# oarodriguez/PhD-QMCLib

Hardware: AMD Instinct MI355X
Metric: walker-steps/sec (higher is better)
Workload: dtype f64

## Files before the change

### phd_qmclib_amd/csrc/qmc_kernels.h

```cpp
#pragma once

#include "qmc_device.h"
#include "qmc_sorted64.h"
#include "qmc_sorted128.h"

#ifndef QMC_SORTED128
#define QMC_SORTED128 1
#endif

static constexpr int BLOCK = 256;

#ifndef QMC_BLOCK64
#define QMC_BLOCK64 64
#endif
template <int G>
struct WalkBlock {
    static constexpr int N = (G == 64) ? QMC_BLOCK64 : BLOCK;
};

#ifndef QMC_XCD_MAP
#define QMC_XCD_MAP 1
#endif
template <int GPB>
__device__ __forceinline__ long long walker_of_block(unsigned b, int grp)
{
    if (QMC_XCD_MAP && GPB == 1)
        return ((long long)(b >> 7) << 7) + ((b & 7u) << 4) + ((b & 127u) >> 3);
    return (long long)b * GPB + grp;
}

template <int G, int P, bool PAD, bool ZC, bool DMC = false>
struct StepLds {
    static constexpr int NROWS =
        DMC ? SortedCot<false, true, false>::ROWS : 5;
    static constexpr int SORTED =
        (QMC_SORTED128 && G == 64 && P == 2 && !ZC)
            ? NROWS * SortedRows<128>::ROW
            : (QMC_SORTED64 && G == 64 && P == 1 && !ZC)
                  ? (NROWS + (QMC_T_LDS ? 1 : 0)) * SortedRows<64>::ROW
                  : 0;
    static constexpr int GENERAL = GroupLds<G, P, ZC>::DOUBLES;
    static constexpr int DOUBLES = SORTED > GENERAL ? SORTED : GENERAL;
};

__device__ __forceinline__ long long qmc_uniform(long long v)
{
    const int lo = __builtin_amdgcn_readfirstlane((int)v);
    const int hi = __builtin_amdgcn_readfirstlane((int)(v >> 32));
    return ((long long)hi << 32) | (unsigned int)lo;
}

#ifndef QMC_LB_P1
#define QMC_LB_P1 7
#endif
#ifndef QMC_LB_DMC_P2
#define QMC_LB_DMC_P2 5
#endif
#define QMC_LB_WAVES , ((G == 64 && P == 1) ? QMC_LB_P1 : 1)
#define QMC_LB_WAVES_DMC , ((G == 64 && P == 1) ? QMC_LB_P1 \
                            : (G == 64 && P == 2 && !ZC) ? QMC_LB_DMC_P2 : 1)
#ifndef QMC_LB_VMC_P2
#define QMC_LB_VMC_P2 4
#endif
#define QMC_LB_WAVES_VMC , ((G == 64 && P == 1) ? QMC_LB_P1 \
                            : (G == 64 && P == 2 && !ZC) ? QMC_LB_VMC_P2 : 1)

#ifndef QMC_VMC_TWO_PASS
#define QMC_VMC_TWO_PASS 1
#endif

#ifndef QMC_DMC_SPARE
#define QMC_DMC_SPARE 1
#endif
template <int P>
struct DmcSpare {
    static constexpr bool ON = QMC_DMC_SPARE && P == 1;
};

#ifndef QMC_RESORT_EVERY
#define QMC_RESORT_EVERY 4
#endif

struct EvalArgs {
    const double *pos;
    double *wf, *energy;
    double *ith, *drift;
    long long nconf;
};

template <int G, int P, bool PAD, bool ZC, typename R = double>
__global__ void __launch_bounds__(WalkBlock<G>::N QMC_LB_WAVES)
evaluate_kernel(const DevModel *__restrict__ mp, EvalArgs a)
{
    const DevModel &m = *mp;
    [[maybe_unused]] constexpr int QMC_SEC_OFF = 0;
    QMC_SECTION("top");
    extern __shared__ double smem[];
    constexpr int GPB = WalkBlock<G>::N / G;
    const int grp = threadIdx.x / G, gl = threadIdx.x % G;
    double *lds = smem + (size_t)grp * GroupLds<G, P, ZC>::DOUBLES;
    const long long w = walker_of_block<GPB>(blockIdx.x, grp);
    const bool active = w < a.nconf;
    if (GPB == 1 && !active) return;
    const long long wr = active ? w : 0;
    const int n = walker_n<G, P, PAD>(m);
    double z[P], z1[P], F[P], ei[P], E, wf;
#pragma unroll
    for (int p = 0; p < P; ++p) {
        int i = lane_particle<G, P, PAD>(m, gl, p);
        z1[p] = (i < n) ? a.pos[wr * n + i] : 0.0;
        z[p] = wrap_box(z1[p], m.L);
    }
    eval_walker<G, P, PAD, true, true, ZC, R>(m, z, z1, gl, lds, F, ei, E, wf);
    if (!active) return;
#pragma unroll
    for (int p = 0; p < P; ++p) {
        int i = lane_particle<G, P, PAD>(m, gl, p);
        if (i < n) {
            if (a.ith) a.ith[w * n + i] = ei[p];
            if (a.drift) a.drift[w * n + i] = F[p];
        }
    }
    if (gl == 0) {
        if (a.wf) a.wf[w] = wf;
        if (a.energy) a.energy[w] = E;
    }
}

struct PrepArgs {
    const double *pos;
    double *drift, *energy;
    long long nconf;
};

template <int G, int P, bool PAD, bool ZC, typename R = double>
__global__ void __launch_bounds__(WalkBlock<G>::N QMC_LB_WAVES)
prepare_kernel(const DevModel *__restrict__ mp, PrepArgs a)
{
    const DevModel &m = *mp;
    [[maybe_unused]] constexpr int QMC_SEC_OFF = 0;
    QMC_SECTION("top");
    extern __shared__ double smem[];
    constexpr int GPB = WalkBlock<G>::N / G;
    const int grp = threadIdx.x / G, gl = threadIdx.x % G;
    double *lds = smem + (size_t)grp * GroupLds<G, P, ZC>::DOUBLES;
    const long long w = walker_of_block<GPB>(blockIdx.x, grp);
    const bool active = w < a.nconf;
    if (GPB == 1 && !active) return;
    const long long wr = active ? w : 0;
    const int n = walker_n<G, P, PAD>(m);
    double z[P], z1[P], F[P], ei[P], E, wf;
#pragma unroll
    for (int p = 0; p < P; ++p) {
        int i = lane_particle<G, P, PAD>(m, gl, p);
        z1[p] = (i < n) ? a.pos[wr * n + i] : 0.0;
        z[p] = wrap_box(z1[p], m.L);
    }
    eval_walker<G, P, PAD, false, false, ZC, R>(m, z, z1, gl, lds, F, ei, E,
                                                wf);
    if (!active) return;
#pragma unroll
    for (int p = 0; p < P; ++p) {
        int i = lane_particle<G, P, PAD>(m, gl, p);
        if (i < n) a.drift[w * n + i] = F[p];
    }
    if (gl == 0) a.energy[w] = E;
}

struct alignas(64) VmcRec {
    double wf;
    double ecarry;
    double sum_e, sum_e2;
    long long n_acc;
    long long spare[3];
};
static_assert(sizeof(VmcRec) == 64, "one record = 8 eight-byte words");
typedef unsigned int VmcRecWords __attribute__((ext_vector_type(16)));
#define QMC_CONST __attribute__((address_space(4)))
__device__ __forceinline__ double vmc_rec_word(const VmcRecWords &r, int k)
{
    return __hiloint2double((int)r[2 * k + 1], (int)r[2 * k]);
}

struct VmcArgs {
    double *pos;
    unsigned short *label;
    VmcRec *rec;
    double *ser_wf, *ser_e;
    unsigned char *ser_stat;
    double *ser_pos;
    const double *tape;
    long long tape_steps;
    long long tape_idx;
    long long W;
    long long y;
    int forced;
    int reset_sums;
    int gaussian;
    unsigned int step;
    unsigned int chain0;
    unsigned long long seed;
    double move_spread;
};

template <int G, int P, bool PAD, bool ZC, bool LEAN, typename R = double,
          bool STEADY = false>
__global__ void __launch_bounds__(WalkBlock<G>::N QMC_LB_WAVES_VMC)
vmc_step_kernel(const DevModel *__restrict__ mp, VmcArgs a)
{
    static_assert(LEAN || !STEADY, "the steady variant is a LEAN kernel");
    const DevModel &m = *mp;
    [[maybe_unused]] constexpr int QMC_SEC_OFF = 0;
    QMC_SECTION("top");
    extern __shared__ double smem[];
    constexpr int GPB = WalkBlock<G>::N / G;
    const int grp = threadIdx.x / G, gl = threadIdx.x % G;
    static_assert(StepLds<G, P, PAD, ZC>::DOUBLES >= GroupLds<G, P, ZC>::DOUBLES,
                  "eval_walker is the fallback on the same LDS region");
    double *lds = smem + (size_t)grp * StepLds<G, P, PAD, ZC>::DOUBLES;
    const long long w = walker_of_block<GPB>(blockIdx.x, grp);
    const bool active = w < a.W;
    if (GPB == 1 && !active) return;
    const long long wr = active ? w : 0;
    const int n = walker_n<G, P, PAD>(m);
    const unsigned int slot = a.chain0 + (unsigned int)wr;
    const bool forced = !STEADY && a.forced != 0;
    const bool reset_sums = !STEADY && a.reset_sums != 0;

    const long long wl = (G == 64) ? qmc_uniform(wr) : wr;
    double wf_cur, e_cur, se = 0.0, se2 = 0.0;
    long long na = 0;
    if constexpr (G == 64) {
        const VmcRecWords r = *(const QMC_CONST VmcRecWords *)(a.rec + wl);
        wf_cur = vmc_rec_word(r, 0);
        e_cur = vmc_rec_word(r, 1);
        se = vmc_rec_word(r, 2);
        se2 = vmc_rec_word(r, 3);
        na = __double_as_longlong(vmc_rec_word(r, 4));
        if (reset_sums) { se = 0.0; se2 = 0.0; na = 0; }
    } else {
        wf_cur = a.rec[wl].wf;
        e_cur = a.rec[wl].ecarry;
    }

    QMC_SECTION("load+philox+wrap");
    double zn[P];
    int labn[P];
    double ua = 1.0;
    unsigned int aw0 = 0u, aw1 = 0u;
    bool has0 = false, has1 = false;
    bool outside = false;
#pragma unroll
    for (int p = 0; p < P; ++p) {
        int i = lane_particle<G, P, PAD>(m, gl, p);
        const double zp = (i < n) ? a.pos[wr * n + i] : 0.0;
        labn[p] = (i < n) ? (int)a.label[wr * n + i] : i;
        const unsigned li = (unsigned)labn[p];
        double d = 0.0;
        if (!forced && i < n) {
            if (!LEAN && a.tape) {
                double tv = a.tape[(wr * a.tape_steps + a.tape_idx) * (n + 1) + li];
                d = a.gaussian ? a.move_spread * tv
                               : (tv - 0.5) * a.move_spread;
            } else if (!LEAN && a.gaussian) {
                double g0, g1;
                philox_normal2(a.seed, slot, a.step, li, STREAM_VMC_MOVE, g0,
                               g1);
                d = a.move_spread * g0;
            } else {
                uint32_t w0, w1;
                vmc_move_block(a.seed, slot, a.step, li, w0, w1);
                d = vmc_move_unit(w0) * a.move_spread;
                if (li == 0u) { aw0 = w1; has0 = true; }
                if (li == 1u || n == 1) { aw1 = w1; has1 = true; }
            }
        }
        zn[p] = wrap_box(zp + d, m.L);
        if (forced) outside = outside || zn[p] != zp;
    }
    QMC_SECTION("resort");
    constexpr bool S64 = QMC_SORTED64 && G == 64 && P == 1 && !ZC;
    constexpr bool S128 = QMC_SORTED128 && G == 64 && P == 2 && !ZC;
    bool fast = false;
    if (forced)
        outside = __builtin_amdgcn_ballot_w64(outside) != 0ull;
    if constexpr (S64) {
        fast = !m.is_ideal && !outside &&
               sort_lanes64(zn[0], labn[0], gl, PAD ? n : 64) &&
               (PAD ? far_partner_ok_ring(m, zn[0], gl, n)
                    : far_partner_ok64(m, zn[0], gl));
    } else if constexpr (S128) {
        fast = !m.is_ideal && !outside && (!PAD || (n & 1) == 0) &&
               sort_rows128(zn, labn, gl, PAD ? n / 2 : 64) &&
               (PAD ? far_partner_ok_ring128(m, zn, gl, n / 2)
                    : far_partner_ok128(m, zn, gl));
    }
    if constexpr (S64 || S128) {
        if (!fast && !m.is_ideal && gl == 0 && active)
            atomicAdd(m.diag, 1ull);
    } else if constexpr (G == 64 && P == 1 && QMC_LINEAR_ORDER) {
        if (!forced) {
            anchor_seam(zn[0], labn[0], n);
            if ((a.step % QMC_RESORT_EVERY) == 0)
                resort_linear<G>(zn[0], labn[0], gl,
                                 a.step / QMC_RESORT_EVERY, n);
        }
    } else if constexpr (SlotMap<G, P>::CONSECUTIVE && QMC_LINEAR_ORDER) {
        if (!forced) {
            anchor_seam_rows<P>(zn, labn, n);
            if ((a.step % QMC_RESORT_EVERY) == 0)
                resort_linear_rows<P>(zn, labn, gl, a.step / QMC_RESORT_EVERY, n);
        }
    } else if (!forced && (a.step % QMC_RESORT_EVERY) == 0)
        resort_step<G, P>(zn, labn, gl, a.step / QMC_RESORT_EVERY, n, m.L,
                          m.half_L, lanes_in_use<G, PAD>(m));
    constexpr bool TWO_PASS = QMC_VMC_TWO_PASS && (G == 64);
    double F[P], ei[P], e_new = 0.0, wf_new;
    if (S64 && fast) {
        if constexpr (S64)
            eval_sorted64<R, true, !TWO_PASS, false, PAD>(
                m, zn[0], gl, lds, F[0], e_new, wf_new);
    } else if (S128 && fast) {
        if constexpr (S128)
            eval_sorted128<R, true, !TWO_PASS, false, PAD>(m, zn, gl, lds, F,
                                                           e_new, wf_new);
    } else {
        double z1[P];
#pragma unroll
        for (int p = 0; p < P; ++p) {
            int i = lane_particle<G, P, PAD>(m, gl, p);
            z1[p] = (outside && i < n) ? a.pos[wr * n + i] : zn[p];
        }
        if constexpr (TWO_PASS)
            eval_walker<G, P, PAD, true, false, ZC, R, false, false>(
                m, zn, z1, gl, lds, F, ei, e_new, wf_new);
        else
            eval_walker<G, P, PAD, true, false, ZC, R>(m, zn, z1, gl, lds, F,
                                                       ei, e_new, wf_new);
    }
    QMC_SECTION("metropolis+store");
    if (!forced) {
        if (!LEAN && a.tape) {
            ua = a.tape[(wr * a.tape_steps + a.tape_idx) * (n + 1) + n];
        } else if (!LEAN && a.gaussian) {
            double u1;
            philox_uniform2(a.seed, slot, a.step, 0u, STREAM_VMC_ACCEPT, ua,
                            u1);
        } else {
            const unsigned long long bal0 = __ballot(has0);
            const unsigned long long bal1 = __ballot(has1);
            unsigned int hi, lo;
            if (G == 64) {
                const int src0 = __builtin_amdgcn_readfirstlane(
                    (int)__ffsll((long long)bal0) - 1) & 63;
                const int src1 = __builtin_amdgcn_readfirstlane(
                    (int)__ffsll((long long)bal1) - 1) & 63;
                hi = (unsigned)__builtin_amdgcn_readlane((int)aw0, src0);
                lo = (unsigned)__builtin_amdgcn_readlane((int)aw1, src1);
            } else {
                const int base = (threadIdx.x & 63) - gl;
                const unsigned long long gmask = (1ull << (G & 63)) - 1ull;
                const int src0 = base + ((__ffsll((long long)((bal0 >> base) &
                                                              gmask)) - 1) & (G - 1));
                const int src1 = base + ((__ffsll((long long)((bal1 >> base) &
                                                              gmask)) - 1) & (G - 1));
                hi = (unsigned)__shfl((int)aw0, src0, 64);
                lo = (unsigned)__shfl((int)aw1, src1, 64);
            }
            ua = u53(hi, lo);
        }
    }
    if (!active) return;
    bool acc = forced || ua <= 0.0 || wf_new > wf_cur;
    if (!acc) acc = wf_new > 0.5 * log_pos(ua) + wf_cur;
    if (G == 64) acc = __builtin_amdgcn_readfirstlane((int)acc) != 0;
    if (acc) {
        if constexpr (TWO_PASS) {
            QMC_SECTION("energy_pass");
            QMC_SECTION_PHASE(QMC_NSEC / 2);
            double wf_unused;
            if (S64 && fast) {
                if constexpr (S64)
                    eval_sorted64<R, false, true, true, PAD>(
                        m, zn[0], gl, lds, F[0], e_new, wf_unused);
            } else if (S128 && fast) {
                if constexpr (S128)
                    eval_sorted128<R, false, true, true, PAD>(
                        m, zn, gl, lds, F, e_new, wf_unused);
            } else {
                double z1[P];
#pragma unroll
                for (int p = 0; p < P; ++p) {
                    int i = lane_particle<G, P, PAD>(m, gl, p);
                    z1[p] = (outside && i < n) ? a.pos[wr * n + i] : zn[p];
                }
                eval_walker<G, P, PAD, false, false, ZC, R, true, true>(
                    m, zn, z1, gl, lds, F, ei, e_new, wf_unused);
            }
            QMC_SECTION_PHASE(0);
            QMC_SECTION("store");
        }
#pragma unroll
        for (int p = 0; p < P; ++p) {
            int i = lane_particle<G, P, PAD>(m, gl, p);
            if (i < n && !forced) {
                a.pos[w * n + i] = zn[p];
                a.label[w * n + i] = (unsigned short)labn[p];
            }
        }
        wf_cur = wf_new;
        e_cur = e_new;
    }
    if (!LEAN && a.ser_pos) {
#pragma unroll
        for (int p = 0; p < P; ++p) {
            int i = lane_particle<G, P, PAD>(m, gl, p);
            if (i < n) {
                const bool moved = acc && !forced;
                const int lb = moved ? labn[p] : (int)a.label[w * n + i];
                a.ser_pos[(a.y * a.W + w) * n + lb] =
                    moved ? zn[p] : a.pos[w * n + i];
            }
        }
    }
    if (G == 64) {
        const double sum1 = se + e_cur;
        const double sum2 = fma(e_cur, e_cur, se2);
        const long long na1 = qmc_uniform(na + (acc ? 1 : 0));
        double v = __longlong_as_double((gl == 4) ? na1 : 0ll);
        v = (gl == 0) ? wf_cur : v;
        v = (gl == 1) ? e_cur : v;
        v = (gl == 2) ? sum1 : v;
        v = (gl == 3) ? sum2 : v;
        if (gl < 8) reinterpret_cast<double *>(a.rec + wl)[gl] = v;
    }
    if (gl == 0) {
        if (G != 64) {
            VmcRec *r = a.rec + w;
            if (!reset_sums) { se = r->sum_e; se2 = r->sum_e2; na = r->n_acc; }
            r->wf = wf_cur;
            r->ecarry = e_cur;
            r->sum_e = se + e_cur;
            r->sum_e2 = fma(e_cur, e_cur, se2);
            r->n_acc = na + (acc ? 1 : 0);
        }
        if (!LEAN) {
            if (a.ser_wf) a.ser_wf[a.y * a.W + w] = wf_cur;
            if (a.ser_e) a.ser_e[a.y * a.W + w] = e_cur;
            if (a.ser_stat) a.ser_stat[a.y * a.W + w] = acc ? 1 : 0;
        }
    }
    QMC_SECTION("end");
}

struct DmcCtl {
    long long prev_nw;
    long long nw;
    double ref_energy;
    double total_energy, total_weight;
    double e_t, w_t;
    long long spare_nw;
    unsigned int step;
    unsigned int pad;
};

struct EvolveArgs {
    const double *ppos, *pdrift, *penergy;
    double *cpos, *cdrift, *cenergy, *cweight;
    const unsigned short *plabel;
    unsigned short *clabel;
    double *eslot;
    const long long *ref;
    const DmcCtl *ctl;
    const double *g_tape;
    double *spare;
    long long maxw;
    double dt, sigma;
    unsigned long long seed;
    unsigned int slot0;
    int fix_stale;
};

template <int G, int P, bool PAD, bool ZC, typename R = double>
__global__ void __launch_bounds__(WalkBlock<G>::N QMC_LB_WAVES_DMC)
dmc_evolve_kernel(const DevModel *__restrict__ mp, EvolveArgs a)
{
    const DevModel &m = *mp;
    [[maybe_unused]] constexpr int QMC_SEC_OFF = 0;
    extern __shared__ double smem[];
    constexpr int GPB = WalkBlock<G>::N / G;
    const int grp = threadIdx.x / G, gl = threadIdx.x % G;
    static_assert(StepLds<G, P, PAD, ZC, true>::DOUBLES >=
                      GroupLds<G, P, ZC>::DOUBLES,
                  "eval_walker is the fallback on the same LDS region");
    double *lds = smem + (size_t)grp * StepLds<G, P, PAD, ZC, true>::DOUBLES;
    const long long s = walker_of_block<GPB>(blockIdx.x, grp);
    const long long nw = a.ctl->nw;
    if ((GPB == 1 ? s : (long long)blockIdx.x * GPB) >= nw) return;
    QMC_SECTION("top");
    const bool active = s < nw;
    const long long sr = active ? s : 0;
    const int n = walker_n<G, P, PAD>(m);
    const unsigned int step = a.ctl->step;
    const double ref_energy = a.ctl->ref_energy;
    const long long spare_nw = a.ctl->spare_nw;
    const long long su = (G == 64) ? qmc_uniform(sr) : sr;
    const long long par = a.ref[su];
    double e_par = 0.0, e_slot = 0.0;
    if (G == 64) {
        e_par = a.penergy[par];
        e_slot = a.eslot[su];
    }

    QMC_SECTION("load+philox+wrap");
    double z[P];
    int lab[P];
#pragma unroll
    for (int p = 0; p < P; ++p) {
        int i = lane_particle<G, P, PAD>(m, gl, p);
        double zz = 0.0;
        lab[p] = i;
        if (i < n) {
            double z0 = a.ppos[par * n + i];
            double f0 = a.pdrift[par * n + i];
            const int li = (int)a.plabel[par * n + i];
            lab[p] = li;
            double g;
            if (a.g_tape) {
                g = a.g_tape[sr * n + li];
            } else if (DmcSpare<P>::ON && (step & 1u) && sr < spare_nw) {
                g = a.spare[sr * n + li];
            } else {
                double g0, g1;
                dmc_normal2(a.seed, a.slot0 + (unsigned)sr, step >> 1,
                            (unsigned)li, g0, g1);
                g = (step & 1u) ? g1 : g0;
                if (DmcSpare<P>::ON && !(step & 1u) && active)
                    a.spare[sr * n + li] = g1;
            }
            double zn = z0 + 2 * f0 * a.dt + a.sigma * g;
            zz = wrap_box(zn, m.L);
        }
        z[p] = zz;
    }
    QMC_SECTION("resort");
    constexpr bool S64 = QMC_SORTED64 && G == 64 && P == 1 && !ZC;
    constexpr bool S128 = QMC_SORTED128 && G == 64 && P == 2 && !ZC;
    bool fast = false;
    if constexpr (S64) {
        fast = !m.is_ideal && sort_lanes64(z[0], lab[0], gl, PAD ? n : 64) &&
               (PAD ? far_partner_ok_ring(m, z[0], gl, n)
                    : far_partner_ok64(m, z[0], gl));
    } else if constexpr (S128) {
        fast = !m.is_ideal && (!PAD || (n & 1) == 0) &&
               sort_rows128(z, lab, gl, PAD ? n / 2 : 64) &&
               (PAD ? far_partner_ok_ring128(m, z, gl, n / 2)
                    : far_partner_ok128(m, z, gl));
    }
    if constexpr (S64 || S128) {
        if (!fast && !m.is_ideal && gl == 0 && active)
            atomicAdd(m.diag, 1ull);
    } else if constexpr (G == 64 && P == 1 && QMC_LINEAR_ORDER) {
        anchor_seam(z[0], lab[0], n);
        if ((step % QMC_RESORT_EVERY) == 0)
            resort_linear<G>(z[0], lab[0], gl, step / QMC_RESORT_EVERY, n);
    } else if constexpr (SlotMap<G, P>::CONSECUTIVE && QMC_LINEAR_ORDER) {
        anchor_seam_rows<P>(z, lab, n);
        if ((step % QMC_RESORT_EVERY) == 0)
            resort_linear_rows<P>(z, lab, gl, step / QMC_RESORT_EVERY, n);
    } else if ((step % QMC_RESORT_EVERY) == 0)
        resort_step<G, P>(z, lab, gl, step / QMC_RESORT_EVERY, n, m.L,
                          m.half_L, lanes_in_use<G, PAD>(m));
#pragma unroll
    for (int p = 0; p < P; ++p) {
        int i = lane_particle<G, P, PAD>(m, gl, p);
        if (active && i < n) {
            a.cpos[s * n + i] = z[p];
            a.clabel[s * n + i] = (unsigned short)lab[p];
        }
    }
    double F[P], ei[P], e_next, wf;
    if (S64 && fast) {
        if constexpr (S64)
            eval_sorted64<R, false, true, false, PAD>(m, z[0], gl, lds, F[0],
                                                      e_next, wf);
    } else if (S128 && fast) {
        if constexpr (S128)
            eval_sorted128<R, false, true, false, PAD>(m, z, gl, lds, F,
                                                       e_next, wf);
    } else
        eval_walker<G, P, PAD, false, false, ZC, R>(m, z, z, gl, lds, F, ei,
                                                    e_next, wf);
    QMC_SECTION("weight+store");
    if (!active) return;
#pragma unroll
    for (int p = 0; p < P; ++p) {
        int i = lane_particle<G, P, PAD>(m, gl, p);
        if (i < n) a.cdrift[s * n + i] = F[p];
    }
    if (gl == 0) {
        if (G != 64) { e_par = a.penergy[par]; e_slot = a.eslot[s]; }
        double e_old = a.fix_stale ? e_par : e_slot;
        double mean_energy = (e_next + e_old) / 2;
// ... 7 lines not shown
```

### phd_qmclib_amd/csrc/qmcwalk.hip

```cpp
#include "qmc_inst.h"
#include "qmc_kernels_misc.h"
#include "../../include/qmcwalk.h"

#include <cmath>
#include <cstdio>
#include <cstdlib>
#include <cstring>
#include <algorithm>
#include <string>
#include <vector>

static thread_local std::string g_err;

static int fail(const std::string &msg)
{
    g_err = msg;
    return 1;
}

#define HIP_TRY(expr)                                                        \
    do {                                                                     \
        hipError_t _e = (expr);                                              \
        if (_e != hipSuccess)                                                \
            return fail(std::string(#expr) + ": " + hipGetErrorString(_e));  \
// ... 50 lines not shown


static int pick_shape(int n, int &G, int &P, bool &pad)
{
    if (n < 1) return 1;
    if (const char *env = getenv("QMCWALK_SHAPE")) {
        int g = 0, p = 0;
        if (sscanf(env, "%d,%d", &g, &p) == 2 && n <= g * p) {
            static const int ok[][2] = { {16, 1}, {16, 2}, {32, 2}, {64, 1},
                                         {64, 2}, {64, 4}, {64, 8} };
            for (auto &s : ok)
                if (s[0] == g && s[1] == p) {
                    G = g; P = p; pad = (n != G * P);
                    return 0;
                }
        }
    }
    if (n <= 16) { G = 16; P = 1; }
    else if (n <= 32) { G = 16; P = 2; }
    else if (n <= 64) { G = 64; P = 1; }
    else if (n <= 128) { G = 64; P = 2; }
    else if (n <= 256) { G = 64; P = 4; }
    else if (n <= 512) { G = 64; P = 8; }
    else return 1;
    pad = (n != G * P);
    return 0;
}

#define QMC_EXTERN_TU(name) QMC_TU_##name(extern)
QMC_FOR_ALL_TUS(QMC_EXTERN_TU)
#undef QMC_EXTERN_TU

template <template <int, int, bool, bool> class L, typename... A>
static int dispatch_shape(const qmc_engine *e, A &&...args)
{
    const bool zc = e->dm.zclass != 0;
#define QMC_CASE(g, p)                                                        \
    if (e->G == g && e->P == p) {                                             \
        constexpr bool always = L<g, p, true, false>::want_mask(p);           \
        if (always || e->pad) {                                               \
            if (zc) return L<g, p, true, true>::run(e, args...);              \
            return L<g, p, true, false>::run(e, args...);                     \
        }                                                                     \
        if constexpr (!always) {                                              \
            if (zc) return L<g, p, false, true>::run(e, args...);             \
            return L<g, p, false, false>::run(e, args...);                    \
        }                                                                     \
    }
    QMC_FOR_ALL_SHAPES(QMC_CASE)
#undef QMC_CASE
    return fail("unsupported boson_number");
}

template <int G, int P, bool ZC>
static size_t lds_bytes()
{
    return (size_t)(WalkBlock<G>::N / G) * GroupLds<G, P, ZC>::DOUBLES *
           sizeof(double);
}

template <int G, int P, bool PAD, bool ZC, bool DMC = false>
static size_t step_lds_bytes()
{
    return (size_t)(WalkBlock<G>::N / G) *
           StepLds<G, P, PAD, ZC, DMC>::DOUBLES * sizeof(double);
}

template <typename K>
static void allow_lds(K kernel, size_t bytes)
{
    if (bytes > 48 * 1024)
        (void)hipFuncSetAttribute((const void *)kernel,
                                  hipFuncAttributeMaxDynamicSharedMemorySize,
                                  (int)bytes);
}

template <int G>
static unsigned grid_for(long long nwalkers)
{
    const long long gpb = WalkBlock<G>::N / G;
    long long blocks = (nwalkers + gpb - 1) / gpb;
    if (QMC_XCD_MAP && gpb == 1) blocks = (blocks + 127) / 128 * 128;
    return (unsigned)blocks;
}

template <int G, bool ZC>
static constexpr bool has_fast() { return G == 64 && !ZC; }

template <int G, int P, bool PAD, bool ZC>
struct LaunchEval {
    static constexpr bool want_mask(int np) { return np >= 4; }
    static int run(const qmc_engine *e, const EvalArgs &a)
    {
        if (a.nconf <= 0) return 0;
        const size_t lds = lds_bytes<G, P, ZC>();
        if constexpr (has_fast<G, ZC>()) {
            if (e->fast) {
                allow_lds(evaluate_kernel<G, P, PAD, ZC, float>, lds);
                hipLaunchKernelGGL((evaluate_kernel<G, P, PAD, ZC, float>),
                                   dim3(grid_for<G>(a.nconf)), dim3(WalkBlock<G>::N),
                                   lds, e->stream, e->dm_dev, a);
                HIP_TRY(hipGetLastError());
                return 0;
            }
        }
        allow_lds(evaluate_kernel<G, P, PAD, ZC>, lds);
        hipLaunchKernelGGL((evaluate_kernel<G, P, PAD, ZC>),
                           dim3(grid_for<G>(a.nconf)), dim3(WalkBlock<G>::N),
                           lds, e->stream, e->dm_dev, a);
        HIP_TRY(hipGetLastError());
        return 0;
    }
};

template <int G, int P, bool PAD, bool ZC>
struct LaunchPrep {
    static constexpr bool want_mask(int np) { return np >= 4; }
    static int run(const qmc_engine *e, const PrepArgs &a)
    {
        if (a.nconf <= 0) return 0;
        const size_t lds = lds_bytes<G, P, ZC>();
        if constexpr (has_fast<G, ZC>()) {
            if (e->fast) {
                allow_lds(prepare_kernel<G, P, PAD, ZC, float>, lds);
                hipLaunchKernelGGL((prepare_kernel<G, P, PAD, ZC, float>),
                                   dim3(grid_for<G>(a.nconf)), dim3(WalkBlock<G>::N),
                                   lds, e->stream, e->dm_dev, a);
                HIP_TRY(hipGetLastError());
                return 0;
            }
        }
        allow_lds(prepare_kernel<G, P, PAD, ZC>, lds);
        hipLaunchKernelGGL((prepare_kernel<G, P, PAD, ZC>),
                           dim3(grid_for<G>(a.nconf)), dim3(WalkBlock<G>::N),
                           lds, e->stream, e->dm_dev, a);
        HIP_TRY(hipGetLastError());
        return 0;
    }
};

template <int G, int P, bool PAD, bool ZC>
struct LaunchVmc {
    static constexpr bool want_mask(int np) { return np >= 4; }
    template <typename R, bool LEAN, bool STEADY>
    static void launch(const qmc_engine *e, const VmcArgs &a, size_t lds)
    {
        allow_lds(vmc_step_kernel<G, P, PAD, ZC, LEAN, R, STEADY>, lds);
        hipLaunchKernelGGL((vmc_step_kernel<G, P, PAD, ZC, LEAN, R, STEADY>),
                           dim3(grid_for<G>(a.W)), dim3(WalkBlock<G>::N), lds,
                           e->stream, e->dm_dev, a);
    }
    template <typename R>
    static void launch(const qmc_engine *e, const VmcArgs &a, size_t lds,
                       bool lean)
    {
        if (lean && !a.forced && !a.reset_sums)
            launch<R, true, true>(e, a, lds);
        else if (lean)
            launch<R, true, false>(e, a, lds);
        else
            launch<R, false, false>(e, a, lds);
    }
    static int run(const qmc_engine *e, const VmcArgs &a)
    {
        const size_t lds = step_lds_bytes<G, P, PAD, ZC>();
        const bool lean = !a.tape && !a.gaussian && !a.ser_wf && !a.ser_e &&
                          !a.ser_stat && !a.ser_pos;
        ProfScope prof(e);
        if constexpr (has_fast<G, ZC>()) {
            if (e->fast) {
                launch<float>(e, a, lds, lean);
                HIP_TRY(hipGetLastError());
                return 0;
            }
        }
        launch<double>(e, a, lds, lean);
        HIP_TRY(hipGetLastError());
        return 0;
    }
};

template <int G, int P, bool PAD, bool ZC>
struct LaunchEvolve {
    static constexpr bool want_mask(int np) { return np >= 4; }
    static int run(const qmc_engine *e, const EvolveArgs &a)
    {
        const size_t lds = step_lds_bytes<G, P, PAD, ZC, true>();
        ProfScope prof(e);
        if constexpr (has_fast<G, ZC>()) {
            if (e->fast) {
                allow_lds(dmc_evolve_kernel<G, P, PAD, ZC, float>, lds);
                hipLaunchKernelGGL((dmc_evolve_kernel<G, P, PAD, ZC, float>),
                                   dim3(grid_for<G>(a.maxw)), dim3(WalkBlock<G>::N),
                                   lds, e->stream, e->dm_dev, a);
                HIP_TRY(hipGetLastError());
                return 0;
            }
        }
        allow_lds(dmc_evolve_kernel<G, P, PAD, ZC>, lds);
        hipLaunchKernelGGL((dmc_evolve_kernel<G, P, PAD, ZC>),
                           dim3(grid_for<G>(a.maxw)), dim3(WalkBlock<G>::N),
                           lds, e->stream, e->dm_dev, a);
        HIP_TRY(hipGetLastError());
        return 0;
    }
};

static void build_dev_model(const qmc_model_params &p, DevModel &d)
{
    memset(&d, 0, sizeof(d));
    d.n = (int)p.boson_number;
    d.is_free = p.is_free != 0;
    d.is_ideal = p.is_ideal != 0;
    d.defects_sep = (int)(p.defects_sep > 0 ? p.defects_sep : 1);
    d.L = p.supercell_size;
    d.half_L = 0.5 * d.L;
    d.rm = fabs(p.tbf_contact_cutoff);
    d.L_minus_rm = d.L - d.rm;
    d.two_over_L = 2.0 / d.L;
    d.k2_2pi = p.param_k2 * (2.0 / QMC_PI);
    d.k2 = p.param_k2;
    d.k2sq = d.k2 * d.k2;
    double phi = p.param_k2 * p.param_r_off;
    d.cphi = cos(phi);
    d.sphi = sin(phi);
    d.sec_cut = -1;
    d.am_cphi = fabs(p.param_am) * d.cphi;
    d.am_sphi = fabs(p.param_am) * d.sphi;
    d.m_k2cphi = -d.k2 * d.cphi;
    d.k2sphi = d.k2 * d.sphi;
    double th = p.param_k2 * d.L;
    d.cth = cos(th);
    d.sth = fabs(sin(th));
    d.sth_sign = sin(th) < 0.0 ? (int)0x80000000u : 0;
    d.sth_signed = sin(th);
    d.sp_ok = (!d.is_ideal && th > 0.0 && th < QMC_PI - 1e-9 &&
               d.rm < d.half_L) ? 1 : 0;
    d.sp_xlo = -d.k2 * sin(d.k2 * d.rm - phi);
    d.sp_xhi = d.k2 * sin(phi);
    d.sp_cos = cos(d.k2 * d.rm);
    {
        const double ang[4] = { -phi, phi, phi - th, th - phi };
        for (int v = 0; v < 4; ++v) {
            d.var_cos[v] = cos(ang[v]);
            d.var_sin[v] = sin(ang[v]);
        }
        d.m_k2 = -d.k2;
    }
    d.sin_rm = (d.rm >= d.half_L) ? 1.0 : sin(QMC_PI * d.rm / d.L);
#ifdef QMC_ABLATION
    if (const char *env = getenv("QMCWALK_ABL_SINRM")) d.sin_rm = atof(env);
#endif
    d.zclass = d.rm > 0.45 * d.L;
    double pi_L = QMC_PI / d.L;
    d.a_long = pi_L * p.param_beta;
    d.b_long = pi_L * pi_L * p.param_beta;
    d.a_long_sq = d.a_long * d.a_long;
    d.m_k2_over_a = d.a_long != 0.0 ? -d.k2 / d.a_long : 0.0;
    d.m_a_over_k2 = d.k2 != 0.0 ? -d.a_long / d.k2 : 0.0;
    d.beta = p.param_beta;
    d.inv_beta = p.param_beta != 0.0 ? 1.0 / p.param_beta : 0.0;
    d.one_minus_beta = 1.0 - p.param_beta;
    d.log_am = log(fabs(p.param_am));
    d.z_a = 1.0 / (1.0 + p.lattice_ratio);
    d.z_b = p.lattice_ratio / (1.0 + p.lattice_ratio);
    d.k1 = p.param_k1;
    d.k1_2pi = p.param_k1 * (2.0 / QMC_PI);
    d.kp1 = p.param_kp1;
    d.e0 = p.param_e0;
    d.v0 = p.lattice_depth;
    d.v0d = p.defect_magnitude;
    d.uniform_barrier = (d.defects_sep == 1 || d.v0d == d.v0) ? 1 : 0;
    d.v_barrier = (d.defects_sep == 1) ? d.v0d : d.v0;
    d.k1_half = 0.5 * p.param_k1;
    d.v0_minus_e0 = p.lattice_depth - p.param_e0;
    if (!d.is_free) {
        double sh = sinh(0.5 * sqrt(d.v0 - d.e0) * d.z_b);
        d.cf = sqrt(1 + d.v0 / d.e0 * sh * sh);
    } else {
        d.cf = 1.0;
    }
}

static void ob_exact(const DevModel &d, long double zc, bool barrier,
                     long double &ldz, long double &logf)
{
    if (barrier) {
        const long double x = (long double)d.kp1 *
                              (zc - 1.0L + 0.5L * (long double)d.z_b);
        ldz = (long double)d.kp1 * tanhl(x);
        logf = logl(coshl(x));
    } else {
        const long double x = (long double)d.k1 *
                              (zc - 0.5L * (long double)d.z_a);
        ldz = -(long double)d.k1 * tanl(x);
        logf = logl((long double)d.cf * cosl(x));
    }
}

template <int DEG, typename F>
static void ob_fit(F f, long double a, long double h, double *coef)
{
    constexpr int K = DEG + 1;
    long double A[K][K + 1];
    for (int j = 0; j < K; ++j) {
        const long double t = 0.5L * (1.0L + cosl(3.14159265358979323846264338L *
                                                  (2 * j + 1) / (2.0L * K)));
        long double pw = 1.0L;
        for (int k = 0; k < K; ++k) { A[j][k] = pw; pw *= t; }
        A[j][K] = f(a + h * t);
    }
    for (int c = 0; c < K; ++c) {
        int piv = c;
        for (int r = c + 1; r < K; ++r)
            if (fabsl(A[r][c]) > fabsl(A[piv][c])) piv = r;
        for (int k = 0; k <= K; ++k) std::swap(A[c][k], A[piv][k]);
        for (int r = c + 1; r < K; ++r) {
            const long double g = A[r][c] / A[c][c];
            for (int k = c; k <= K; ++k) A[r][k] -= g * A[c][k];
        }
    }
    for (int r = K - 1; r >= 0; --r) {
        long double v = A[r][K];
        for (int k = r + 1; k < K; ++k) v -= A[r][k] * (long double)coef[k];
        coef[r] = (double)(v / A[r][r]);
    }
}

static double ob_horner(const double *c, int deg, double t)
// ... 680 lines not shown
                       v->ecarry);
    HIP_TRY(hipGetLastError());
    HIP_TRY(hipStreamSynchronize(e->stream));
    v->step = 0;
    v->yield_initial = 1;
    v->tape_used = 0;
    return 0;
}

extern "C" int qmc_vmc_get_state(qmc_vmc *v, double *pos, double *wf,
                                 double *ecarry)
{
    if (!v) return fail("qmc_vmc_get_state: null argument");
    qmc_engine *e = v->eng;
    HIP_TRY(hipSetDevice(e->device));
    const size_t W = (size_t)v->W, n = (size_t)e->dm.n;
    std::vector<double> lane_pos;
    std::vector<unsigned short> label;
    if (pos) {
        lane_pos.resize(W * n);
        label.resize(W * n);
        HIP_TRY(hipMemcpyAsync(lane_pos.data(), v->pos, W * n * sizeof(double),
                               hipMemcpyDeviceToHost, e->stream));
        HIP_TRY(hipMemcpyAsync(label.data(), v->label,
                               W * n * sizeof(unsigned short),
                               hipMemcpyDeviceToHost, e->stream));
    }
    if (wf) HIP_TRY(hipMemcpyAsync(wf, v->wf, W * sizeof(double),
                                   hipMemcpyDeviceToHost, e->stream));
    if (ecarry) HIP_TRY(hipMemcpyAsync(ecarry, v->ecarry, W * sizeof(double),
                                       hipMemcpyDeviceToHost, e->stream));
    HIP_TRY(hipStreamSynchronize(e->stream));
    if (pos)
        for (size_t w = 0; w < W; ++w)
            for (size_t i = 0; i < n; ++i)
                pos[w * n + label[w * n + i]] = lane_pos[w * n + i];
    return 0;
}

extern "C" int qmc_vmc_set_tape(qmc_vmc *v, const double *tape, int64_t steps)
{
    if (!v) return fail("qmc_vmc_set_tape: null argument");
    qmc_engine *e = v->eng;
    HIP_TRY(hipSetDevice(e->device));
    if (v->tape) { hipFree(v->tape); v->tape = nullptr; }
    v->tape_steps = 0;
    v->tape_used = 0;
    if (!tape || steps <= 0) return 0;
    size_t cnt = (size_t)v->W * (size_t)steps * (size_t)(e->dm.n + 1);
    if (dev_alloc(&v->tape, cnt)) return 1;
    HIP_TRY(hipMemcpy(v->tape, tape, cnt * sizeof(double),
                      hipMemcpyHostToDevice));
    v->tape_steps = steps;
    return 0;
}

extern "C" int qmc_vmc_state_dev(qmc_vmc *v, double **pos, double **wf)
{
    if (!v) return fail("null argument");
    if (pos) *pos = v->pos;
    if (wf) *wf = v->wf;
    return 0;
}

extern "C" int qmc_vmc_ssf(qmc_vmc *v, int32_t num_modes, double *out)
{
    if (!v || !out) return fail("qmc_vmc_ssf: null argument");
    if (num_modes <= 0 || num_modes > EST_MAXK)
        return fail("qmc_vmc_ssf: num_modes must be in [1, 256]");
    qmc_engine *e = v->eng;
    HIP_TRY(hipSetDevice(e->device));
    const int M = num_modes;
    if (M > v->ssf_cap) {
        if (v->ssf_partial) { hipFree(v->ssf_partial); hipFree(v->ssf_out); }
        v->ssf_partial = v->ssf_out = nullptr;
        if (dev_alloc(&v->ssf_partial, (size_t)EST_BLOCKS * M * 3) ||
            dev_alloc(&v->ssf_out, (size_t)M * 3))
            return 1;
        v->ssf_cap = M;
    }
    EstArgs a;
    a.ppos = v->pos; a.ref = nullptr; a.ctl = nullptr;
    a.aux_prev = nullptr; a.aux_act = nullptr; a.partial = v->ssf_partial;
    a.maxw = v->W; a.step_idx = 0; a.pfw = 0; a.n = e->dm.n; a.K = M;
    a.pure = 0; a.scale = 4.0 / e->dm.L;
    if (M <= 64) {
        const size_t lds = (size_t)(BLOCK / 64) * SsfShape<8>::WAVE_DOUBLES *
                           sizeof(double);
        allow_lds(dmc_ssf_mfma_kernel<8>, lds);
        hipLaunchKernelGGL(dmc_ssf_mfma_kernel<8>, dim3(EST_BLOCKS),
                           dim3(BLOCK), lds, e->stream, a);
    } else {
        const size_t lds = (size_t)(BLOCK / 64) * SsfShape<16>::WAVE_DOUBLES *
                           sizeof(double);
        allow_lds(dmc_ssf_mfma_kernel<16>, lds);
        hipLaunchKernelGGL(dmc_ssf_mfma_kernel<16>, dim3(EST_BLOCKS),
                           dim3(BLOCK), lds, e->stream, a);
    }
    hipLaunchKernelGGL(est_reduce_kernel, dim3((M * 3 + 31) / 32), dim3(256), 0,
                       e->stream, v->ssf_partial, EST_BLOCKS, M * 3, 1.0,
                       v->ssf_out);
    HIP_TRY(hipGetLastError());
    HIP_TRY(hipMemcpyAsync(out, v->ssf_out, (size_t)M * 3 * sizeof(double),
                           hipMemcpyDeviceToHost, e->stream));
    HIP_TRY(hipStreamSynchronize(e->stream));
    return 0;
}

extern "C" int qmc_vmc_block_sums_dev(qmc_vmc *v, double **se, double **se2,
                                      int64_t **na)
{
    if (!v) return fail("null argument");
    if (se) *se = v->sum_e;
    if (se2) *se2 = v->sum_e2;
    if (na) *na = (int64_t *)v->n_acc;
    return 0;
}

extern "C" int qmc_vmc_run_block(qmc_vmc *v, int64_t nyield, double *sum_e,
                                 double *sum_e2, int64_t *n_acc,
                                 double *ser_wf, double *ser_e,
                                 uint8_t *ser_stat, double *ser_pos)
{
    if (!v) return fail("qmc_vmc_run_block: null argument");
    if (nyield <= 0) return fail("qmc_vmc_run_block: nyield must be >= 1");
    qmc_engine *e = v->eng;
    HIP_TRY(hipSetDevice(e->device));
    const size_t W = (size_t)v->W, ny = (size_t)nyield;
    const long long real = nyield - (v->yield_initial ? 1 : 0);
    if (v->tape && v->tape_used + real > v->tape_steps)
        return fail("qmc_vmc_run_block: tape exhausted");
    double *dwf = nullptr, *de = nullptr;
    unsigned char *dst = nullptr;
    double *dpos = nullptr;
    if ((ser_pos && dev_alloc(&dpos, ny * W * (size_t)e->dm.n)) ||
        (ser_wf && dev_alloc(&dwf, ny * W)) ||
        (ser_e && dev_alloc(&de, ny * W)) ||
        (ser_stat && dev_alloc(&dst, ny * W))) {
        if (dpos) hipFree(dpos);
        if (dwf) hipFree(dwf);
        if (de) hipFree(de);
        if (dst) hipFree(dst);
        return 1;
    }
    VmcArgs a;
    a.pos = v->pos; a.label = v->label; a.rec = v->rec;
    a.ser_wf = dwf; a.ser_e = de; a.ser_stat = dst; a.ser_pos = dpos;
    a.tape = v->tape;
    a.tape_steps = v->tape_steps;
    a.W = v->W;
    a.gaussian = v->p.gaussian;
    a.chain0 = v->p.chain0;
    a.seed = v->p.rng_seed; a.move_spread = v->p.move_spread;
    for (long long y = 0; y < nyield; ++y) {
        a.y = y;
        a.forced = (y == 0 && v->yield_initial) ? 1 : 0;
        a.reset_sums = (y == 0) ? 1 : 0;
        a.step = v->step;
        a.tape_idx = v->tape_used;
        int rc = dispatch_shape<LaunchVmc>(e, a);
        if (rc) return rc;
        if (!a.forced) { v->step += 1; v->tape_used += 1; }
    }
    v->yield_initial = 0;
    hipLaunchKernelGGL(vmc_unpack_kernel, dim3((unsigned)((W + BLOCK - 1) / BLOCK)),
                       dim3(BLOCK), 0, e->stream, v->rec, v->W, v->wf, v->ecarry,
                       v->sum_e, v->sum_e2, v->n_acc);
    HIP_TRY(hipGetLastError());
    bool need_sync = false;
    if (sum_e) { HIP_TRY(hipMemcpyAsync(sum_e, v->sum_e, W * sizeof(double),
                 hipMemcpyDeviceToHost, e->stream)); need_sync = true; }
    if (sum_e2) { HIP_TRY(hipMemcpyAsync(sum_e2, v->sum_e2, W * sizeof(double),
                  hipMemcpyDeviceToHost, e->stream)); need_sync = true; }
    if (n_acc) { HIP_TRY(hipMemcpyAsync(n_acc, v->n_acc, W * sizeof(int64_t),
                 hipMemcpyDeviceToHost, e->stream)); need_sync = true; }
    if (ser_wf) { HIP_TRY(hipMemcpyAsync(ser_wf, dwf, ny * W * sizeof(double),
                  hipMemcpyDeviceToHost, e->stream)); need_sync = true; }
    if (ser_e) { HIP_TRY(hipMemcpyAsync(ser_e, de, ny * W * sizeof(double),
                 hipMemcpyDeviceToHost, e->stream)); need_sync = true; }
    if (ser_stat) { HIP_TRY(hipMemcpyAsync(ser_stat, dst, ny * W,
                    hipMemcpyDeviceToHost, e->stream)); need_sync = true; }
    if (ser_pos) { HIP_TRY(hipMemcpyAsync(ser_pos, dpos,
                   ny * W * (size_t)e->dm.n * sizeof(double),
                   hipMemcpyDeviceToHost, e->stream)); need_sync = true; }
    if (need_sync) HIP_TRY(hipStreamSynchronize(e->stream));
    if (dpos) hipFree(dpos);
    if (dwf) hipFree(dwf);
    if (de) hipFree(de);
    if (dst) hipFree(dst);
    return 0;
}

struct qmc_dmc {
    qmc_engine *eng = nullptr;
    qmc_dmc_params p;
    long long maxw = 0;
    int nblocks = 0;
    double *pos[2] = { nullptr, nullptr }, *drift[2] = { nullptr, nullptr };
    unsigned short *label[2] = { nullptr, nullptr };
    double *energy[2] = { nullptr, nullptr }, *weight[2] = { nullptr, nullptr };
    int cur = 0;
    double *eslot = nullptr;
    double *spare = nullptr;
    long long *ref = nullptr;
    int *count = nullptr;
    long long *block_tot = nullptr, *block_off = nullptr;
    double *block_esum = nullptr;
    DmcCtl *ctl = nullptr;
    double *ser_e = nullptr, *ser_w = nullptr, *ser_ref = nullptr,
           *ser_acc = nullptr;
    unsigned long long *ser_nw = nullptr;
    long long ser_cap = 0, ser_len = 0;
    double *u_tape = nullptr, *g_tape = nullptr;
    std::vector<long long> u_off, g_off;
    long long tape_step = 0;
    bool stepped = false;
    std::vector<double> init_weight;
    bool sums_pending = false;
    double global_target = 0.0;
    qmc_dmc_est_params est;
    bool have_est = false;
    double *ssf_aux[2] = { nullptr, nullptr };
    double *dens_aux[2] = { nullptr, nullptr };
    double *est_partial = nullptr;
    double *iter_ssf = nullptr, *iter_dens = nullptr;
    size_t iter_ssf_cap = 0, iter_dens_cap = 0;
    long long est_block_steps = 0;
    int est_last_act = 1;
};

static int dmc_reserve_series(qmc_dmc *d, long long nsteps)
{
    if (nsteps <= d->ser_cap) return 0;
    if (d->ser_e) hipFree(d->ser_e);
    if (d->ser_w) hipFree(d->ser_w);
    if (d->ser_ref) hipFree(d->ser_ref);
    if (d->ser_acc) hipFree(d->ser_acc);
    if (d->ser_nw) hipFree(d->ser_nw);
    d->ser_e = d->ser_w = d->ser_ref = d->ser_acc = nullptr;
    d->ser_nw = nullptr;
    d->ser_cap = 0;
    if (dev_alloc(&d->ser_e, nsteps) || dev_alloc(&d->ser_w, nsteps) ||
        dev_alloc(&d->ser_ref, nsteps) || dev_alloc(&d->ser_acc, nsteps) ||
        dev_alloc(&d->ser_nw, nsteps)) {
        if (d->ser_e) hipFree(d->ser_e);
        if (d->ser_w) hipFree(d->ser_w);
        if (d->ser_ref) hipFree(d->ser_ref);
        if (d->ser_acc) hipFree(d->ser_acc);
        if (d->ser_nw) hipFree(d->ser_nw);
        d->ser_e = d->ser_w = d->ser_ref = d->ser_acc = nullptr;
        d->ser_nw = nullptr;
        return 1;
    }
    d->ser_cap = nsteps;
    return 0;
}

extern "C" void qmc_dmc_destroy(qmc_dmc *d);

extern "C" int qmc_dmc_create(qmc_engine *e, const qmc_dmc_params *p,
                              qmc_dmc **out)
{
    if (!e || !p || !out) return fail("qmc_dmc_create: null argument");
    if (p->max_num_walkers <= 0 || p->target_num_walkers <= 0)
        return fail("qmc_dmc_create: walker counts must be positive");
    if (!(p->time_step > 0)) return fail("qmc_dmc_create: time_step <= 0");
    HIP_TRY(hipSetDevice(e->device));
    qmc_dmc *d = new qmc_dmc();
    d->eng = e;
    d->p = *p;
    d->maxw = p->max_num_walkers;
    d->nblocks = (int)((d->maxw + BR_TILE - 1) / BR_TILE);
    d->global_target = (double)p->target_num_walkers;
    const size_t W = (size_t)d->maxw, n = (size_t)e->dm.n;
    int rc = 0;
    for (int b = 0; b < 2 && !rc; ++b) {
        rc |= dev_alloc(&d->pos[b], W * n) || dev_alloc(&d->drift[b], W * n) ||
              dev_alloc(&d->label[b], W * n) ||
              dev_alloc(&d->energy[b], W) || dev_alloc(&d->weight[b], W);
    }
    const bool need_spare = QMC_DMC_SPARE && e->P == 1;
    rc = rc || dev_alloc(&d->eslot, W) ||
         (need_spare && dev_alloc(&d->spare, W * n)) ||
         dev_alloc(&d->ref, W) ||
         dev_alloc(&d->count, W) || dev_alloc(&d->block_tot, d->nblocks) ||
         dev_alloc(&d->block_off, d->nblocks) ||
         dev_alloc(&d->block_esum, d->nblocks) || dev_alloc(&d->ctl, 1);
    if (rc) { qmc_dmc_destroy(d); return 1; }
    HIP_TRY(hipMemset(d->ctl, 0, sizeof(DmcCtl)));
    HIP_TRY(hipMemset(d->ref, 0, W * sizeof(long long)));
    HIP_TRY(hipMemset(d->eslot, 0, W * sizeof(double)));
    *out = d;
    return 0;
}

extern "C" void qmc_dmc_destroy(qmc_dmc *d)
{
    if (!d) return;
    hipSetDevice(d->eng->device);
    for (int b = 0; b < 2; ++b) {
        hipFree(d->pos[b]); hipFree(d->drift[b]); hipFree(d->label[b]);
        hipFree(d->energy[b]); hipFree(d->weight[b]);
    }
    hipFree(d->eslot); hipFree(d->spare); hipFree(d->ref); hipFree(d->count);
    hipFree(d->block_tot); hipFree(d->block_off); hipFree(d->block_esum);
    hipFree(d->ctl);
    if (d->ser_e) { hipFree(d->ser_e); hipFree(d->ser_w); hipFree(d->ser_ref);
                    hipFree(d->ser_acc); hipFree(d->ser_nw); }
    if (d->u_tape) hipFree(d->u_tape);
    if (d->g_tape) hipFree(d->g_tape);
    for (int k = 0; k < 2; ++k) {
        if (d->ssf_aux[k]) hipFree(d->ssf_aux[k]);
        if (d->dens_aux[k]) hipFree(d->dens_aux[k]);
    }
    if (d->est_partial) hipFree(d->est_partial);
// ... 798 lines not shown
```

Before: 711.0 million.

## Fuse steady-state VMC steps into one kernel launch with register-resident walker state

In the steady lean VMC path, one kernel launch now runs all remaining steps for a walker in a loop. Positions, labels, energy and accumulator sums stay in registers across steps and are written back to global memory only once at the end. The acceptance random words are taken from the lanes holding labels 0 and 1 using precomputed source lanes and readlane, instead of a ballot on every step. This removes the per-step launch overhead and the per-step global load/store of walker state, at the cost of longer-running kernels, more register pressure, and an opaque-asm trick to keep the compiler from hoisting work out of the loop.

Measured after the change: 762.7 million, median of 6. 1.07x the previous value.

```diff
diff --git a/phd_qmclib_amd/csrc/qmc_kernels.h b/phd_qmclib_amd/csrc/qmc_kernels.h
--- a/phd_qmclib_amd/csrc/qmc_kernels.h
+++ b/phd_qmclib_amd/csrc/qmc_kernels.h
@@ -48,6 +48,49 @@
     const int lo = __builtin_amdgcn_readfirstlane((int)v);
     const int hi = __builtin_amdgcn_readfirstlane((int)(v >> 32));
     return ((long long)hi << 32) | (unsigned int)lo;
+}
+__device__ __forceinline__ int qmc_opaque(int v)
+{
+    asm volatile("" : "+v"(v));
+    return v;
+}
+__device__ __forceinline__ double qmc_uniform_f64(double v)
+{
+    return __longlong_as_double(qmc_uniform(__double_as_longlong(v)));
+}
+__device__ __forceinline__ double qmc_lane_f64(double v, int k)
+{
+    const long long b = __double_as_longlong(v);
+    const int lo = __builtin_amdgcn_readlane((int)b, k);
+    const int hi = __builtin_amdgcn_readlane((int)(b >> 32), k);
+    return __longlong_as_double(((long long)hi << 32) | (unsigned int)lo);
+}
+
+template <int P>
+__device__ __forceinline__ void vmc_accept_lanes(const int (&lab)[P], int n,
+                                                 int &src0, int &src1)
+{
+    src0 = 0;
+    src1 = 0;
+#pragma unroll
+    for (int p = 0; p < P; ++p) {
+        const unsigned long long b0 = __ballot(lab[p] == 0);
+        const unsigned long long b1 = __ballot(lab[p] == 1);
+        if (b0) src0 = ((int)__ffsll((long long)b0) - 1) | (p << 6);
+        if (b1) src1 = ((int)__ffsll((long long)b1) - 1) | (p << 6);
+    }
+    if (n == 1) src1 = src0;
+}
+template <int P>
+__device__ __forceinline__ unsigned int vmc_read_slot(const uint32_t (&wd)[P],
+                                                      int src)
+{
+    unsigned int r = 0u;
+#pragma unroll
+    for (int p = 0; p < P; ++p)
+        if ((src >> 6) == p)
+            r = (unsigned)__builtin_amdgcn_readlane((int)wd[p], src & 63);
+    return r;
 }
 
 #ifndef QMC_LB_P1
@@ -194,6 +237,7 @@
     long long tape_idx;
     long long W;
     long long y;
+    unsigned int nsteps;
     int forced;
     int reset_sums;
     int gaussian;
@@ -201,6 +245,16 @@
     unsigned int chain0;
     unsigned long long seed;
     double move_spread;
+};
+
+#ifndef QMC_VMC_FUSED
+#define QMC_VMC_FUSED 1
+#endif
+template <int G, int P, bool ZC>
+struct VmcFused {
+    static constexpr bool ON =
+        QMC_VMC_FUSED && G == 64 && !ZC &&
+        ((P == 1 && QMC_SORTED64) || (P == 2 && QMC_SORTED128));
 };
 
 template <int G, int P, bool PAD, bool ZC, bool LEAN, typename R = double,
@@ -243,6 +297,26 @@
         e_cur = a.rec[wl].ecarry;
     }
 
+    constexpr bool FUSED = STEADY && VmcFused<G, P, ZC>::ON;
+    double zc[P];
+    int labc[P];
+    int src0 = 0, src1 = 0;
+    if constexpr (FUSED) {
+#pragma unroll
+        for (int p = 0; p < P; ++p) {
+            int i = lane_particle<G, P, PAD>(m, gl, p);
+            zc[p] = (i < n) ? a.pos[wr * n + i] : 0.0;
+            labc[p] = (i < n) ? (int)a.label[wr * n + i] : i;
+        }
+        vmc_accept_lanes<P>(labc, n, src0, src1);
+    }
+    bool any_acc = false;
+    const unsigned int nst = FUSED ? a.nsteps : 1u;
+    bool acc = false;
+    [[maybe_unused]] const int gl_top = gl;
+    for (unsigned int s = 0; s < nst; ++s) {
+    const unsigned int step = a.step + s;
+    const int gl = FUSED ? qmc_opaque(gl_top) : gl_top;
     QMC_SECTION("load+philox+wrap");
     double zn[P];
     int labn[P];
@@ -250,11 +324,19 @@
     unsigned int aw0 = 0u, aw1 = 0u;
     bool has0 = false, has1 = false;
     bool outside = false;
-#pragma unroll
-    for (int p = 0; p < P; ++p) {
+    [[maybe_unused]] uint32_t wacc[P];
+#pragma unroll
+    for (int p = 0; p < P; ++p) {
+        wacc[p] = 0u;
         int i = lane_particle<G, P, PAD>(m, gl, p);
-        const double zp = (i < n) ? a.pos[wr * n + i] : 0.0;
-        labn[p] = (i < n) ? (int)a.label[wr * n + i] : i;
+        double zp;
+        if constexpr (FUSED) {
+            zp = zc[p];
+            labn[p] = labc[p];
+        } else {
+            zp = (i < n) ? a.pos[wr * n + i] : 0.0;
+            labn[p] = (i < n) ? (int)a.label[wr * n + i] : i;
+        }
         const unsigned li = (unsigned)labn[p];
         double d = 0.0;
         if (!forced && i < n) {
@@ -264,19 +346,27 @@
                                : (tv - 0.5) * a.move_spread;
             } else if (!LEAN && a.gaussian) {
                 double g0, g1;
-                philox_normal2(a.seed, slot, a.step, li, STREAM_VMC_MOVE, g0,
+                philox_normal2(a.seed, slot, step, li, STREAM_VMC_MOVE, g0,
                                g1);
                 d = a.move_spread * g0;
             } else {
                 uint32_t w0, w1;
-                vmc_move_block(a.seed, slot, a.step, li, w0, w1);
+                vmc_move_block(a.seed, slot, step, li, w0, w1);
                 d = vmc_move_unit(w0) * a.move_spread;
-                if (li == 0u) { aw0 = w1; has0 = true; }
-                if (li == 1u || n == 1) { aw1 = w1; has1 = true; }
+                if constexpr (FUSED) {
+                    wacc[p] = w1;
+                } else {
+                    if (li == 0u) { aw0 = w1; has0 = true; }
+                    if (li == 1u || n == 1) { aw1 = w1; has1 = true; }
+                }
             }
         }
         zn[p] = wrap_box(zp + d, m.L);
         if (forced) outside = outside || zn[p] != zp;
+    }
+    if constexpr (FUSED) {
+        aw0 = vmc_read_slot<P>(wacc, src0);
+        aw1 = vmc_read_slot<P>(wacc, src1);
     }
     QMC_SECTION("resort");
     constexpr bool S64 = QMC_SORTED64 && G == 64 && P == 1 && !ZC;
@@ -339,12 +429,14 @@
                                                        ei, e_new, wf_new);
     }
     QMC_SECTION("metropolis+store");
-    if (!forced) {
+    if (FUSED) {
+        ua = u53(aw0, aw1);
+    } else if (!forced) {
         if (!LEAN && a.tape) {
             ua = a.tape[(wr * a.tape_steps + a.tape_idx) * (n + 1) + n];
         } else if (!LEAN && a.gaussian) {
             double u1;
-            philox_uniform2(a.seed, slot, a.step, 0u, STREAM_VMC_ACCEPT, ua,
+            philox_uniform2(a.seed, slot, step, 0u, STREAM_VMC_ACCEPT, ua,
                             u1);
         } else {
             const unsigned long long bal0 = __ballot(has0);
@@ -371,9 +463,16 @@
         }
     }
     if (!active) return;
-    bool acc = forced || ua <= 0.0 || wf_new > wf_cur;
-    if (!acc) acc = wf_new > 0.5 * log_pos(ua) + wf_cur;
-    if (G == 64) acc = __builtin_amdgcn_readfirstlane((int)acc) != 0;
+    if constexpr (FUSED) {
+        const double w0 = qmc_uniform_f64(wf_new);
+        acc = ua <= 0.0 || w0 > wf_cur;
+        if (!acc) acc = w0 > 0.5 * log_pos(ua) + wf_cur;
+        acc = __builtin_amdgcn_readfirstlane((int)acc) != 0;
+    } else {
+        acc = forced || ua <= 0.0 || wf_new > wf_cur;
+        if (!acc) acc = wf_new > 0.5 * log_pos(ua) + wf_cur;
+        if (G == 64) acc = __builtin_amdgcn_readfirstlane((int)acc) != 0;
+    }
     if (acc) {
         if constexpr (TWO_PASS) {
             QMC_SECTION("energy_pass");
@@ -400,16 +499,45 @@
             QMC_SECTION_PHASE(0);
             QMC_SECTION("store");
         }
-#pragma unroll
-        for (int p = 0; p < P; ++p) {
-            int i = lane_particle<G, P, PAD>(m, gl, p);
-            if (i < n && !forced) {
-                a.pos[w * n + i] = zn[p];
-                a.label[w * n + i] = (unsigned short)labn[p];
+        if constexpr (FUSED) {
+#pragma unroll
+            for (int p = 0; p < P; ++p) {
+                zc[p] = zn[p];
+                labc[p] = labn[p];
             }
-        }
-        wf_cur = wf_new;
-        e_cur = e_new;
+            vmc_accept_lanes<P>(labc, n, src0, src1);
+            any_acc = true;
+        } else {
+#pragma unroll
+            for (int p = 0; p < P; ++p) {
+                int i = lane_particle<G, P, PAD>(m, gl, p);
+                if (i < n && !forced) {
+                    a.pos[w * n + i] = zn[p];
+                    a.label[w * n + i] = (unsigned short)labn[p];
+                }
+            }
+        }
+        if (!FUSED) {
+            wf_cur = wf_new;
+            e_cur = e_new;
+        }
+    }
+    if constexpr (FUSED) {
+        if (acc) {
+            wf_cur = qmc_uniform_f64(wf_new);
+            const double e2 = qmc_lane_f64(e_new, 2);
+            const double e3 = qmc_lane_f64(e_new, 3);
+            e_cur = qmc_lane_f64(e_new, 1);
+            se = se + e2;
+            se2 = fma(e3, e3, se2);
+            na = na + 1;
+        } else {
+            se = se + e_cur;
+            se2 = fma(e_cur, e_cur, se2);
+        }
+        se = qmc_uniform_f64(se);
+        se2 = qmc_uniform_f64(se2);
+        continue;
     }
     if (!LEAN && a.ser_pos) {
 #pragma unroll
@@ -449,6 +577,26 @@
             if (a.ser_e) a.ser_e[a.y * a.W + w] = e_cur;
             if (a.ser_stat) a.ser_stat[a.y * a.W + w] = acc ? 1 : 0;
         }
+    }
+    }
+    if constexpr (FUSED) {
+        QMC_SECTION("fused_store");
+        if (any_acc) {
+#pragma unroll
+            for (int p = 0; p < P; ++p) {
+                int i = lane_particle<G, P, PAD>(m, gl, p);
+                if (i < n) {
+                    a.pos[w * n + i] = zc[p];
+                    a.label[w * n + i] = (unsigned short)labc[p];
+                }
+            }
+        }
+        double v = __longlong_as_double((gl == 4) ? qmc_uniform(na) : 0ll);
+        v = (gl == 0) ? wf_cur : v;
+        v = (gl == 1) ? e_cur : v;
+        v = (gl == 2) ? se : v;
+        v = (gl == 3) ? se2 : v;
+        if (gl < 8) reinterpret_cast<double *>(a.rec + wl)[gl] = v;
     }
     QMC_SECTION("end");
 }
diff --git a/phd_qmclib_amd/csrc/qmcwalk.hip b/phd_qmclib_amd/csrc/qmcwalk.hip
--- a/phd_qmclib_amd/csrc/qmcwalk.hip
+++ b/phd_qmclib_amd/csrc/qmcwalk.hip
@@ -226,29 +226,31 @@
     }
     template <typename R>
     static void launch(const qmc_engine *e, const VmcArgs &a, size_t lds,
-                       bool lean)
+                       bool lean, bool steady)
     {
-        if (lean && !a.forced && !a.reset_sums)
+        if (steady)
             launch<R, true, true>(e, a, lds);
         else if (lean)
             launch<R, true, false>(e, a, lds);
         else
             launch<R, false, false>(e, a, lds);
     }
-    static int run(const qmc_engine *e, const VmcArgs &a)
+    static int run(const qmc_engine *e, const VmcArgs &a, long long *ran)
     {
         const size_t lds = step_lds_bytes<G, P, PAD, ZC>();
         const bool lean = !a.tape && !a.gaussian && !a.ser_wf && !a.ser_e &&
                           !a.ser_stat && !a.ser_pos;
+        const bool steady = lean && !a.forced && !a.reset_sums;
+        *ran = (steady && VmcFused<G, P, ZC>::ON) ? (long long)a.nsteps : 1;
         ProfScope prof(e);
         if constexpr (has_fast<G, ZC>()) {
             if (e->fast) {
-                launch<float>(e, a, lds, lean);
+                launch<float>(e, a, lds, lean, steady);
                 HIP_TRY(hipGetLastError());
                 return 0;
             }
         }
-        launch<double>(e, a, lds, lean);
+        launch<double>(e, a, lds, lean, steady);
         HIP_TRY(hipGetLastError());
         return 0;
     }
@@ -1235,15 +1237,18 @@
     a.gaussian = v->p.gaussian;
     a.chain0 = v->p.chain0;
     a.seed = v->p.rng_seed; a.move_spread = v->p.move_spread;
-    for (long long y = 0; y < nyield; ++y) {
+    for (long long y = 0; y < nyield;) {
         a.y = y;
         a.forced = (y == 0 && v->yield_initial) ? 1 : 0;
         a.reset_sums = (y == 0) ? 1 : 0;
         a.step = v->step;
         a.tape_idx = v->tape_used;
-        int rc = dispatch_shape<LaunchVmc>(e, a);
+        a.nsteps = (unsigned int)(nyield - y);
+        long long ran = 1;
+        int rc = dispatch_shape<LaunchVmc>(e, a, &ran);
         if (rc) return rc;
-        if (!a.forced) { v->step += 1; v->tape_used += 1; }
+        if (!a.forced) { v->step += ran; v->tape_used += ran; }
+        y += ran;
     }
     v->yield_initial = 0;
     hipLaunchKernelGGL(vmc_unpack_kernel, dim3((unsigned)((W + BLOCK - 1) / BLOCK)),
```
